# fmidev/RoadSurf

Measured on AMD Instinct MI355X. Metric: point_timesteps_per_s, higher is better.
Workload: dtype f64

## Files before the change

### roadsurf_amd/csrc/rs_api.hip

```cpp
#include <hip/hip_runtime.h>
#include <atomic>
#include <cmath>
#include <cstdarg>
#include <cstdio>
#include <cstdlib>
#include <cstring>
#include <mutex>
#include <utility>
#include <vector>

#include "../../include/roadsurf.h"
#include "rs_kernels.h"
#include "rs_devutil.hpp"
#include <cstdint>
#include <algorithm>
#include "rs_consts_dev.h"
#include "rs_state.h"

static thread_local char g_err[512] = "";

static int set_err(const char *fmt, ...) {
  va_list ap;
  va_start(ap, fmt);
  vsnprintf(g_err, sizeof(g_err), fmt, ap);
// ... 28 lines not shown
  double *relax_tab = nullptr;
  double *cpl_tab = nullptr;
  void *consts32_dev = nullptr;
  rs::Writeback wb{nullptr, nullptr, nullptr, 0};
  int32_t *cpl_flags = nullptr, *cpl_list = nullptr, *cpl_count = nullptr;
  void *cpl_tmp = nullptr;
  size_t cpl_tmp_bytes = 0;
  int32_t cpl_rounds_last = 0;
  bool output_by_point = false;
  bool cpl_windows_closed = false;
  bool history_score = true;
  bool f32 = false;
  double *diag = nullptr;
  bool diag_on = false;
  bool resorted = false;
  int32_t *wave_tab = nullptr;
  int32_t wave_n = 0;
  bool wave_tab_valid = false;
  std::vector<void *> owned;
  rsu::Arena *arena = nullptr;
  uint64_t arena_epoch = 0;
  bool arena_set = false;
  std::vector<hipEvent_t> ev;
  size_t ev_used = 0;
  bool timing = false;
};

template <class T>
static hipError_t plan_malloc(RsPlan *pl, T **p, size_t bytes) {
  rsu::Arena *a = rsu::tls_arena();
// ... 203 lines not shown

static inline int32_t underfilled(const RsPlan *pl) {
  return g_live_points[pl->device & 63].load() <= 131072 ? 1 : 0;
}

void rs_hip_plan_destroy(RsPlan *pl) {
  if (!pl) return;
  g_live_points[pl->device & 63] -= pl->npoints;
  (void)hipSetDevice(pl->device);
  (void)hipStreamSynchronize(pl->stream);
  for (hipEvent_t e : pl->ev) (void)hipEventDestroy(e);
  for (void *q : pl->owned) (void)hipFree(q);
  delete pl;
}

const int32_t *rs_hip_plan_order(RsPlan *pl) {
  if (!pl) {
    set_err("rs_hip_plan_order: null plan");
    return nullptr;
  }
  if (!pl->order) {
    if (hipSetDevice(pl->device) != hipSuccess ||
        plan_malloc(pl, &pl->order, pl->np_pad * sizeof(int32_t)) != hipSuccess ||
        rs_cluster_identity(pl->order, pl->np_pad, pl->stream) != hipSuccess) {
      set_err("rs_hip_plan_order: allocation failed");
      return nullptr;
    }
  }
  return pl->order;
}

static int recluster_buffers(RsPlan *pl) {
  const size_t state_bytes = (size_t)RS_NSTATE * pl->np_pad * sizeof(double);
  if (!pl->state_alt) {
    HIP_OK(plan_malloc(pl, &pl->state_alt, state_bytes));
    HIP_OK(plan_malloc(pl, &pl->order_alt, pl->np_pad * sizeof(int32_t)));
    HIP_OK(plan_malloc(pl, &pl->sort_keys, (size_t)4 * pl->np_pad * sizeof(uint32_t)));
    pl->sort_tmp_bytes = std::max(rs_cluster_scratch_bytes(pl->npoints),
                                  rs_cluster_count_scratch_bytes(pl->npoints, 12));
    HIP_OK(plan_malloc(pl, &pl->sort_tmp, pl->sort_tmp_bytes ? pl->sort_tmp_bytes : 8));
  }
  return 0;
}

static int recluster_apply(RsPlan *pl) {
  pl->resorted = true;
  HIP_OK(rs_cluster_apply(pl->state, pl->state_alt, pl->f32, pl->order, pl->order_alt,
                          pl->sort_keys + 3 * pl->np_pad, pl->np_pad, pl->npoints, pl->c.NLayers,
                          pl->c.use_coupling == 0 ? 0 : pl->cpl_windows_closed ? 1 : 2, pl->stream));
  std::swap(pl->state, pl->state_alt);
  std::swap(pl->order, pl->order_alt);
  return 0;
}

int rs_hip_recluster_forecast(RsPlan *pl, const RsPreview *pv) {
  if (!pl || !pv) return set_err("rs_hip_recluster_forecast: bad arguments");
  if (pv->n < 1 || pv->n > RS_PREVIEW_MAX || (!pv->tair_now && !pv->tair_b[0]))
    return set_err("rs_hip_recluster_forecast: 1 <= n <= %d previews and tair_now (or a preview 0 between two rows) are required",
                   RS_PREVIEW_MAX);
  for (int q = 0; q < pv->n; ++q) {
    if (!pv->tair[q] || !pv->vz[q]) return set_err("rs_hip_recluster_forecast: preview row %d is null", q);
    if ((pv->tair_b[q] != nullptr) != (pv->vz_b[q] != nullptr) || (pv->tair_b[q] && !(pv->w[q] >= 0.0 && pv->w[q] <= 1.0)))
      return set_err("rs_hip_recluster_forecast: preview %d: tair_b and vz_b come together, with 0 <= w <= 1", q);
  }
  if (pl->diag_on)
    return set_err("rs_hip_recluster_forecast: a plan with diagnostics keeps its order (rs_hip_set_diagnostics)");
// ... 30 lines not shown
        HIP_OK(plan_malloc(pl, &pl->wave_tab, ((size_t)2 * maxw + 64) * sizeof(int32_t)));
        pl->wave_n = maxw;
        HIP_OK(hipMemsetAsync(pl->wave_tab + 2 * (size_t)maxw, 0, 64 * sizeof(int32_t), pl->stream));
      }
      class_total = reinterpret_cast<uint32_t *>(pl->wave_tab + 2 * (size_t)maxw);
    }
    HIP_OK(rs_cluster_count_sort(pl->np_pad, pl->npoints, bits, pl->sort_keys, pl->sort_tmp,
                                 pl->sort_tmp_bytes, pl->stream, class_total, cb, low));
    if (table) {
      HIP_OK(rs_cluster_wave_table(cb, class_total, pl->wave_tab, pl->wave_tab + maxw, maxw, pl->stream));
      pl->wave_tab_valid = true;
    }
  } else
    HIP_OK(rs_cluster_sort_keys(pl->np_pad, pl->npoints, pl->sort_keys, pl->sort_tmp, pl->sort_tmp_bytes,
                                pl->stream));
  return recluster_apply(pl);
}

int rs_hip_recluster(RsPlan *pl) {
  if (!pl) return set_err("rs_hip_recluster: null plan");
  if (!pl->history_score)
    return set_err("rs_hip_recluster: the plan's history score is switched off (rs_hip_set_history_score)");
  if (pl->diag_on) return set_err("rs_hip_recluster: a plan with diagnostics keeps its order (rs_hip_set_diagnostics)");
  if (!rs_hip_plan_order(pl)) return -1;
  pl->wave_tab_valid = false;
  HIP_OK(hipSetDevice(pl->device));
  if (recluster_buffers(pl)) return -1;
  HIP_OK(rs_cluster_sort(pl->state, pl->f32, pl->np_pad, pl->npoints, pl->sort_keys, pl->sort_tmp,
                         pl->sort_tmp_bytes, pl->stream));
  return recluster_apply(pl);
}

int rs_hip_plan_order_copy(RsPlan *pl, int32_t *dst) {
  if (!pl || !dst) return set_err("rs_hip_plan_order_copy: bad arguments");
  if (!rs_hip_plan_order(pl)) return -1;
  HIP_OK(hipSetDevice(pl->device));
  HIP_OK(hipMemcpyAsync(dst, pl->order, (size_t)pl->np_pad * sizeof(int32_t), hipMemcpyDeviceToDevice,
                        pl->stream));
  return 0;
}

int rs_hip_outputs_by_point(RsPlan *pl, const RsOutputs *src, int32_t nrows, const int32_t *order,
                            double *const *dst, int64_t dst_rows, int64_t dst_row0, void *stream) {
  if (!pl || !src || !dst || nrows < 1 || dst_rows < 1 || dst_row0 < 0 || dst_row0 + nrows > dst_rows)
    return set_err("rs_hip_outputs_by_point: bad arguments (rows [dst_row0, dst_row0 + nrows) must lie inside a point's dst_rows)");
  if (pl->f32) return set_err("rs_hip_outputs_by_point: fp64 output windows only");
  const double *in[6] = {src->tsurf, src->snow, src->water, src->ice, src->deposit, src->ice2};
  double *out[6];
  for (int f = 0; f < 6; ++f) {
    if (!in[f] || !dst[f]) return set_err("rs_hip_outputs_by_point: all six streams are required on both sides");
    out[f] = dst[f];
  }
  if (src->t_stride < pl->npoints) return set_err("rs_hip_outputs_by_point: t_stride below the plan's points");
  if (!order && stream) return set_err("rs_hip_outputs_by_point: on a stream of the caller's the order row must be a kept one");
  if (!order && !rs_hip_plan_order(pl)) return -1;
  HIP_OK(hipSetDevice(pl->device));
  HIP_OK(rs_cluster_outputs_by_point(in, out, order ? order : pl->order, pl->npoints, src->t_stride, nrows, dst_rows,
                                     dst_row0, stream ? (hipStream_t)stream : pl->stream));
  return 0;
}

int rs_hip_plan_reset_order(RsPlan *pl) {
  if (!pl) return set_err("rs_hip_plan_reset_order: null plan");
  pl->wave_tab_valid = false;
  if (!pl->order) return rs_hip_plan_order(pl) ? 0 : -1;
  HIP_OK(hipSetDevice(pl->device));
  HIP_OK(rs_cluster_identity(pl->order, pl->np_pad, pl->stream));
  pl->resorted = false;
  return 0;
}

int64_t rs_hip_plan_npoints(const RsPlan *pl) { return pl ? pl->npoints : 0; }
int64_t rs_hip_plan_npoints_padded(const RsPlan *pl) { return pl ? pl->np_pad : 0; }
size_t rs_hip_plan_state_bytes(const RsPlan *pl) {
  return pl ? (size_t)RS_NSTATE * pl->np_pad * sizeof(double) : 0;
}

int rs_hip_set_precision(RsPlan *pl, int32_t bits) {
  if (!pl || (bits != 32 && bits != 64)) return set_err("rs_hip_set_precision: bits must be 32 or 64");
  HIP_OK(hipSetDevice(pl->device));
  if (bits == 32) {
    if (!pl->consts32_dev) HIP_OK(plan_malloc(pl, &pl->consts32_dev, rs32_constants_bytes()));
    HIP_OK(rs32_upload_constants(pl->consts32_dev, &pl->c, pl->stream));
  }
  pl->f32 = (bits == 32);
  return 0;
}

int rs_hip_set_writeback(RsPlan *pl, double *sw, double *sw_dir, double *lw, int64_t t_stride) {
  if (!pl) return set_err("rs_hip_set_writeback: null plan");
  if ((sw || sw_dir || lw) && (!sw || !sw_dir || !lw || t_stride < pl->npoints))
    return set_err("rs_hip_set_writeback: all three streams and t_stride >= npoints, or all NULL");
  pl->wb = rs::Writeback{sw, sw_dir, lw, t_stride};
  return 0;
}

int rs_hip_set_diagnostics(RsPlan *pl, int32_t on) {
  if (!pl) return set_err("rs_hip_set_diagnostics: null plan");
  if (on && pl->f32) return set_err("rs_hip_set_diagnostics: the fp64 flavour only");
  if (on && pl->resorted)
    return set_err("rs_hip_set_diagnostics: the block is kept by slot - not for a plan that has been re-sorted");
  HIP_OK(hipSetDevice(pl->device));
  if (on) {
    const size_t bytes = (size_t)RS_DIAG_ROWS * pl->np_pad * sizeof(double);
    if (!pl->diag) HIP_OK(plan_malloc(pl, &pl->diag, bytes));
    HIP_OK(hipMemsetAsync(pl->diag, 0, bytes, pl->stream));
  }
  pl->diag_on = on != 0;
  return 0;
}

int rs_hip_diagnostics(RsPlan *pl, double *out) {
  if (!pl || !out) return set_err("rs_hip_diagnostics: bad arguments");
  if (!pl->diag_on || !pl->diag) return set_err("rs_hip_diagnostics: rs_hip_set_diagnostics(plan, 1) first");
  HIP_OK(hipSetDevice(pl->device));
  std::vector<double> rows((size_t)(RS_DIAG_ROWS + 1) * pl->np_pad);
  HIP_OK(hipMemcpyAsync(rows.data(), pl->diag, (size_t)RS_DIAG_ROWS * pl->np_pad * sizeof(double), hipMemcpyDeviceToHost,
                        pl->stream));
  HIP_OK(hipMemcpyAsync(rows.data() + (size_t)RS_DIAG_ROWS * pl->np_pad, pl->state + (size_t)RS_ST_CPL_FLAGS * pl->np_pad,
                        (size_t)pl->np_pad * sizeof(double), hipMemcpyDeviceToHost, pl->stream));
  HIP_OK(hipStreamSynchronize(pl->stream));
  for (int64_t p = 0; p < pl->npoints; ++p) {
    for (int r = 0; r < RS_DIAG_ROWS; ++r) out[(size_t)p * RS_DIAG_COLS + r] = rows[(size_t)r * pl->np_pad + p];
    const int32_t fl = (int32_t)rows[(size_t)RS_DIAG_ROWS * pl->np_pad + p];
    out[(size_t)p * RS_DIAG_COLS + RS_DIAG_ROWS] = (double)(fl & (RS_CPL_MSG_SMALL | RS_CPL_MSG_BIG));
  }
  return 0;
}

int rs_hip_set_output_by_point(RsPlan *pl, int32_t on) {
  if (!pl) return set_err("rs_hip_set_output_by_point: null plan");
  pl->output_by_point = on != 0;
  return 0;
}

int rs_hip_coupling_windows_closed(RsPlan *pl, int32_t closed) {
  if (!pl) return set_err("rs_hip_coupling_windows_closed: null plan");
  pl->cpl_windows_closed = closed != 0;
  return 0;
}

int rs_hip_set_history_score(RsPlan *pl, int32_t on) {
  if (!pl) return set_err("rs_hip_set_history_score: null plan");
  pl->history_score = on != 0;
  return 0;
}

int rs_hip_set_variant(RsPlan *pl, int32_t variant) {
  if (!pl || variant < 0 || variant > 4) return set_err("rs_hip_set_variant: the flavour is 0 (automatic) ... 4");
  if (variant == RS_VARIANT_REG && pl->c.NLayers != 15)
    return set_err("register-profile kernel is built for NLayers == 15 only (got %d)",
                   pl->c.NLayers);
// ... 1 lines not shown
  return 0;
}

static int check_forcing(const RsPlan *pl, const RsForcing *f, const char *who) {
  if (!f || !f->tair || !f->vz || !f->rhz || !f->prec || !f->sw || !f->lw || !f->precphase ||
      !f->hour)
    return set_err("%s: forcing streams tair,vz,rhz,prec,sw,lw,precphase,hour are required", who);
  if (f->t_stride < pl->npoints)
    return set_err("%s: forcing t_stride %lld < npoints %lld", who, (long long)f->t_stride,
                   (long long)pl->npoints);
  return 0;
}

int rs_hip_init_state(RsPlan *pl, const RsForcing *f, const RsPointParams *pp) {
  if (!pl) return set_err("rs_hip_init_state: null plan");
  if (check_forcing(pl, f, "rs_hip_init_state")) return -1;
  if (!pp || !pp->tbottom) return set_err("rs_hip_init_state: tbottom is required");
  HIP_OK(hipSetDevice(pl->device));
  rs::InitArgs a;
  a.consts = pl->f32 ? pl->consts32_dev : pl->consts_dev;
  a.f = *f;
  a.pp = *pp;
  a.state = pl->state;
  a.npoints = pl->npoints;
  a.np_pad = pl->np_pad;
  pl->cpl_windows_closed = false;
  if (pl->f32) {
    HIP_OK(rs32_launch_init(a, pl->stream));
  } else {
    HIP_OK(rs_launch_init(a, pl->stream));
// ... 39 lines not shown
      HIP_OK(rs_cpl_select_again(pl->state, pl->np_pad, pl->npoints, pl->cpl_flags, pl->cpl_list,
                                 pl->cpl_count, pl->cpl_tmp, pl->cpl_tmp_bytes, pl->stream));
      HIP_OK(hipMemcpyAsync(&n_again, pl->cpl_count, sizeof(n_again), hipMemcpyDeviceToHost, pl->stream));
      HIP_OK(hipStreamSynchronize(pl->stream));
      if (n_again != 0)
        return set_err("coupling replays: %d points still ask for a replay after 64 rounds - the window "
                       "passed does not cover their coupling windows", n_again);
    }
  }
  return 0;
}

int rs_hip_step(RsPlan *pl, const RsForcing *f, const RsOutputs *o, const RsPointParams *pp,
                int32_t t0, int32_t nsteps) {
  if (!pl) return set_err("rs_hip_step: null plan");
  if (check_forcing(pl, f, "rs_hip_step")) return -1;
  if (!pp || !pp->tbottom) return set_err("rs_hip_step: tbottom is required");
  if (!o || !o->tsurf || !o->snow || !o->water || !o->ice || !o->deposit || !o->ice2)
    return set_err("rs_hip_step: all six output streams are required");
  if (o->t_stride < pl->npoints) return set_err("rs_hip_step: output t_stride < npoints");
  if (o->decimate < 1) return set_err("rs_hip_step: decimate must be >= 1");
  if (t0 < 1 || nsteps < 1 || (int64_t)t0 + nsteps - 1 > pl->c.SimLen)
    return set_err("rs_hip_step: window [%d,%d) outside [1,SimLen=%d]", t0, t0 + nsteps,
                   pl->c.SimLen);
  {
    const int64_t first = ((int64_t)t0 - 1 + o->decimate - 1) / o->decimate;
    if (first < o->row0) return set_err("rs_hip_step: output row0 %lld beyond first row %lld",
                                        (long long)o->row0, (long long)first);
  }
  HIP_OK(hipSetDevice(pl->device));
// ... 44 lines not shown
  a.duo_full_ok = (full && !skyview && !coupled && !f->depth && !(pl->c.tsurfOutputDepth >= 0.0)) ? 1 : 0;
  {
    const int64_t orows = ((int64_t)t0 + nsteps - 2) / o->decimate - o->row0 + 1;
    const bool a32 = (uint64_t)f->t_stride * (uint64_t)nsteps < rs_a32_limit() &&
                     (uint64_t)o->t_stride * (uint64_t)(orows > 0 ? orows : 1) < rs_a32_limit() &&
                     (!pl->wb.sw_dir || (uint64_t)pl->wb.t_stride * (uint64_t)nsteps < rs_a32_limit());
    if (skyview && !coupled && !f->depth && !(pl->c.tsurfOutputDepth >= 0.0) && a32) a.duo_full_ok |= 4;
  }
  a.surface_prio = underfilled(pl);
  a.knots = nullptr;
  a.knot_gather = nullptr;
  a.knot_k0 = a.knot_n = a.spk = a.start_hour = 0;
  a.r_spk = 0.0;
  std::memset(&a.raw, 0, sizeof(a.raw));
  a.diag = pl->diag_on ? pl->diag : nullptr;
  hipEvent_t e0 = nullptr, e1 = nullptr;
  if (pl->timing) {
    if (pl->ev_used + 2 > pl->ev.size()) {
      hipEvent_t x, y;
      HIP_OK(hipEventCreate(&x));
      if (hipEventCreate(&y) != hipSuccess) {
        (void)hipEventDestroy(x);
        return set_err("rs_hip_step: hipEventCreate failed");
      }
      pl->ev.push_back(x);
      pl->ev.push_back(y);
    }
    e0 = pl->ev[pl->ev_used];
    e1 = pl->ev[pl->ev_used + 1];
    HIP_OK(hipEventRecord(e0, pl->stream));
// ... 43 lines not shown
    const int32_t klast = tlast / spk + ((tlast % spk) ? 1 : 0);
    if (kfirst < k0 || klast >= k0 + nknots)
      return set_err("rs_hip_step_knots: need knots %d..%d, buffer has %d..%d", kfirst, klast, k0, k0 + nknots - 1);
    const int64_t first = ((int64_t)t0 - 1 + o->decimate - 1) / o->decimate;
    if (first < o->row0) return set_err("rs_hip_step_knots: output row0 beyond first row");
  }
  const int64_t out_rows = ((int64_t)t0 + nsteps - 2) / o->decimate - o->row0 + 1;
  if (pl->c.NLayers != 15 || pl->c.tsurfOutputDepth >= 0.0 || pp->sky_view ||
      (pl->c.use_coupling && pp->coupling_index) ||
      (!pl->f32 && (uint64_t)o->t_stride * (uint64_t)(out_rows > 0 ? out_rows : 1) >= rs_a32_limit()))
    return set_err("rs_hip_step_knots: NLayers = 15, no output depth, sky view or coupling and (fp64) an output "
                   "window below 4 GiB per stream only - use rs_hip_expand_forcing_ordered + rs_hip_step");
  const bool full = (pp->initlen != nullptr) || pl->c.force_tsurf || (pl->c.use_relaxation && pp->tair_relax != nullptr);
  if (pl->c.use_relaxation && pp->tair_relax && (!pp->vz_relax || !pp->rh_relax || !pp->initlen))
    return set_err("rs_hip_step_knots: relaxation needs tair_relax, vz_relax, rh_relax and initlen");
  const int32_t *order = rs_hip_plan_order(pl);
  if (!order) return -1;
  HIP_OK(hipSetDevice(pl->device));
  rs::StepArgs a;
  std::memset(&a, 0, sizeof(a));
  a.consts = pl->f32 ? pl->consts32_dev : pl->consts_dev;
  a.f.t_stride = pl->np_pad;
  a.o = *o;
  a.pp = *pp;
  a.state = pl->state;
  a.npoints = pl->npoints;
  a.np_pad = pl->np_pad;
  a.t0 = t0;
  a.nsteps = nsteps;
  a.wave_start = pl->wave_tab_valid ? pl->wave_tab : nullptr;
  a.wave_cnt = pl->wave_tab_valid ? pl->wave_tab + pl->wave_n : nullptr;
  a.wave_n = pl->wave_n;
  a.duo_full_ok = full ? 3 : 0;
  a.surface_prio = underfilled(pl);
  a.knots = knots;
  a.knot_gather = order;
  a.knot_k0 = k0;
  a.knot_n = nknots;
  a.spk = spk;
  a.start_hour = spec->start_hour;
  a.r_spk = 1.0 / (double)spk;
  a.diag = nullptr;
  hipEvent_t e0 = nullptr, e1 = nullptr;
  if (pl->timing) {
    if (pl->ev_used + 2 > pl->ev.size()) {
      hipEvent_t x, y;
      HIP_OK(hipEventCreate(&x));
      if (hipEventCreate(&y) != hipSuccess) {
        (void)hipEventDestroy(x);
        return set_err("rs_hip_step_knots: hipEventCreate failed");
      }
      pl->ev.push_back(x);
      pl->ev.push_back(y);
    }
    e0 = pl->ev[pl->ev_used];
    e1 = pl->ev[pl->ev_used + 1];
    HIP_OK(hipEventRecord(e0, pl->stream));
  }
  const hipError_t le = pl->f32 ? rs32_launch_step_knots(a, pl->history_score, full, pl->stream)
                                : rs_launch_step_duo_knots(a, pl->history_score, pl->stream);
  if (le != hipSuccess) return set_err("rs_hip_step_knots: kernel launch failed: %s", hipGetErrorString(le));
  if (pl->timing) {
    HIP_OK(hipEventRecord(e1, pl->stream));
    pl->ev_used += 2;
  }
  return 0;
}

}

int rs_step_raw(RsPlan *pl, const rs::RawForcing *raw, const double *sun, const RsOutputs *o,
                const RsPointParams *pp, int32_t t0, int32_t nsteps, bool out_by_point) {
  if (!pl || !raw || raw->nsrc < 1 || raw->nsrc > RS_MAX_SOURCES || !raw->segs || !raw->hour)
    return set_err("rs_step_raw: bad arguments");
  if (!pp || !pp->tbottom || !pp->initlen) return set_err("rs_step_raw: tbottom and initlen are required");
  if (!o || !o->tsurf || !o->snow || !o->water || !o->ice || !o->deposit || !o->ice2)
    return set_err("rs_step_raw: all six output streams are required");
  if (o->t_stride < pl->npoints || o->decimate < 1) return set_err("rs_step_raw: bad output window");
  if (t0 < 1 || nsteps < 1 || (int64_t)t0 + nsteps - 1 > pl->c.SimLen)
    return set_err("rs_step_raw: window [%d,%d) outside [1,SimLen=%d]", t0, t0 + nsteps, pl->c.SimLen);
  const int64_t first = ((int64_t)t0 - 1 + o->decimate - 1) / o->decimate;
  if (first < o->row0) return set_err("rs_step_raw: output row0 beyond first row");
  const int64_t out_rows = ((int64_t)t0 + nsteps - 2) / o->decimate - o->row0 + 1;
  if (!rs_step_raw_ok(pl) || (uint64_t)o->t_stride * (uint64_t)(out_rows > 0 ? out_rows : 1) >= rs_a32_limit())
    return set_err("rs_step_raw: NLayers = 15, fp64, no output depth and an output window below 4 GiB per stream only");
  const bool coupled = pl->c.use_coupling != 0;
  if (coupled && (!pp->coupling_index || !pp->coupling_tsurf))
    return set_err("rs_step_raw: use_coupling is set: pass coupling_index and coupling_tsurf");
  if (pl->c.use_relaxation && pp->tair_relax && (!pp->vz_relax || !pp->rh_relax))
// ... 20 lines not shown
  a.wave_n = pl->wave_n;
  a.duo_full_ok = 3;
  a.surface_prio = underfilled(pl);
  a.raw = *raw;
  a.diag = nullptr;
  a.out_index = (out_by_point && pl->order) ? pl->order : nullptr;
  const hipError_t le = rs_launch_step_duo_raw(a, pl->history_score, sky, coupled, pl->stream);
  if (le != hipSuccess) return set_err("rs_step_raw: kernel launch failed: %s", hipGetErrorString(le));
  return 0;
}

int rs_cpl_replay_raw(RsPlan *pl, const rs::RawForcing *raw, const RsOutputs *o, const RsPointParams *pp,
                      int32_t t0, int32_t nsteps, bool out_by_point, int32_t *rounds) {
  if (!pl || !raw || raw->nsrc < 1 || raw->nsrc > RS_MAX_SOURCES || !raw->segs || !raw->hour)
    return set_err("rs_cpl_replay_raw: bad arguments");
  if (!pp || !pp->tbottom || !pp->initlen || !pp->coupling_index || !pp->coupling_tsurf)
    return set_err("rs_cpl_replay_raw: tbottom, initlen, coupling_index and coupling_tsurf are required");
  if (!pl->c.use_coupling || !rs_step_raw_ok(pl) || pp->sky_view)
    return set_err("rs_cpl_replay_raw: a coupled plan with NLayers = 15, fp64, no output depth, no sky view only");
  if (!o || !o->tsurf || !o->snow || !o->water || !o->ice || !o->deposit || !o->ice2 || o->decimate < 1)
    return set_err("rs_cpl_replay_raw: all six output streams are required");
  if (t0 < 1 || nsteps < 1 || (int64_t)t0 + nsteps - 1 >= pl->c.SimLen)
    return set_err("rs_cpl_replay_raw: the block [%d,%d] must lie inside [1, SimLen - 1]", t0, t0 + nsteps - 1);
  const int64_t out_rows = ((int64_t)t0 + nsteps - 2) / o->decimate - o->row0 + 1;
  if ((uint64_t)o->t_stride * (uint64_t)(out_rows > 0 ? out_rows : 1) >= rs_a32_limit())
    return set_err("rs_cpl_replay_raw: output window of 4 GiB per stream or more");
  if (raw->seg0 < 0 || raw->seg0 >= raw->nseg) return set_err("rs_cpl_replay_raw: seg0 outside the segment table");
  HIP_OK(hipSetDevice(pl->device));
  rs::StepArgs a;
  std::memset(&a, 0, sizeof(a));
// ... 29 lines not shown
  }
  if (cpl_replay_rounds(pl, a, true, true)) return -1;
  if (rounds) *rounds = pl->cpl_rounds_last;
  return 0;
}

bool rs_step_raw_ok(const RsPlan *pl) {
  return pl && !pl->f32 && pl->c.NLayers == 15 && !(pl->c.tsurfOutputDepth >= 0.0);
}

extern "C" {

static int cpl_args(RsPlan *pl, const RsForcing *f, const RsOutputs *o, const RsPointParams *pp,
                    int32_t t0, int32_t nsteps, const char *who, rs::StepArgs &a) {
  if (!pl) return set_err("%s: null plan", who);
  if (check_forcing(pl, f, who)) return -1;
  if (!pp || !pp->tbottom || !pp->coupling_index || !pp->coupling_tsurf)
    return set_err("%s: tbottom, coupling_index and coupling_tsurf are required", who);
  if (!pl->c.use_coupling) return set_err("%s: the plan's settings have use_coupling = 0", who);
  if (pl->f32) return set_err("%s: time-chunked coupling needs the fp64 flavour (an fp32 plan runs a coupled series whole: rs_hip_step)", who);
  if (pp->sky_view) {
    if (!pp->sin_lat || !pp->cos_lat || !pp->lon_rad || !f->sw_dir || !f->lw_net || !f->sun)
      return set_err("%s: sky view needs sin_lat, cos_lat, lon_rad, sw_dir, lw_net and sun", who);
    if (f->hour_pstride) return set_err("%s: sky view needs a time axis shared by all points", who);
    if (pl->wb.sw_dir)
      return set_err("%s: the write-back of the sky-view edits follows whole-series windows: use "
                     "rs_hip_step", who);
  }
  if (pl->c.use_relaxation && pp->tair_relax && (!pp->vz_relax || !pp->rh_relax || !pp->initlen))
    return set_err("%s: relaxation needs tair_relax, vz_relax, rh_relax and initlen", who);
// ... 15 lines not shown
  a.cpl_list = nullptr;
  a.cpl_nlist = 0;
  a.cpl_stop = 0;
  a.cpl_inner = a.cpl_prio = 0;
  a.out_index = (pl->output_by_point && pl->order) ? pl->order : nullptr;
  a.wave_start = a.wave_cnt = nullptr;
  a.wave_n = 0;
  a.duo_full_ok = 0;
  a.surface_prio = 0;
  a.diag = nullptr;
  a.knots = nullptr;
  a.knot_gather = nullptr;
  a.knot_k0 = a.knot_n = a.spk = a.start_hour = 0;
  a.r_spk = 0.0;
  std::memset(&a.raw, 0, sizeof(a.raw));
  return 0;
}

int rs_hip_step_cpl(RsPlan *pl, const RsForcing *f, const RsOutputs *o, const RsPointParams *pp,
                    int32_t t0, int32_t nsteps) {
  rs::StepArgs a;
  if (cpl_args(pl, f, o, pp, t0, nsteps, "rs_hip_step_cpl", a)) return -1;
  HIP_OK(hipSetDevice(pl->device));
  HIP_OK(rs_launch_step_cpl(a, pl->c.NLayers, pl->stream));
  return 0;
}

int rs_hip_cpl_replay(RsPlan *pl, const RsForcing *f, const RsOutputs *o, const RsPointParams *pp,
                      int32_t t0, int32_t nsteps, int32_t *rounds) {
  rs::StepArgs a;
// ... 61 lines not shown
  if (hipEventSynchronize(pl->ev[pl->ev_used - 1]) != hipSuccess) return -1;
  for (int32_t i = 0; i < n && i < cap; ++i) {
    float a = 0.f, b = 0.f;
    if (hipEventElapsedTime(&a, (hipEvent_t)ref_event, pl->ev[2 * (size_t)i]) != hipSuccess ||
        hipEventElapsedTime(&b, (hipEvent_t)ref_event, pl->ev[2 * (size_t)i + 1]) != hipSuccess)
      return set_err("rs_hip_timing_intervals: hipEventElapsedTime failed");
    start_ms[i] = a;
    stop_ms[i] = b;
  }
  return n;
}

int rs_hip_state_download(RsPlan *pl, double *host, size_t bytes) {
  if (!pl || !host || bytes != rs_hip_plan_state_bytes(pl))
    return set_err("rs_hip_state_download: bad arguments");
  HIP_OK(hipSetDevice(pl->device));
  HIP_OK(hipMemcpyAsync(host, pl->state, bytes, hipMemcpyDeviceToHost, pl->stream));
  HIP_OK(hipStreamSynchronize(pl->stream));
  return 0;
}

int rs_hip_state_upload(RsPlan *pl, const double *host, size_t bytes) {
  if (!pl || !host || bytes != rs_hip_plan_state_bytes(pl))
    return set_err("rs_hip_state_upload: bad arguments");
  HIP_OK(hipSetDevice(pl->device));
  HIP_OK(hipMemcpyAsync(pl->state, host, bytes, hipMemcpyHostToDevice, pl->stream));
  HIP_OK(hipStreamSynchronize(pl->stream));
  return 0;
}

int rs_hip_clock_probe(int32_t device, void *out, uint32_t spin_us, void *stream) {
  if (!out) return set_err("rs_hip_clock_probe: null output");
  HIP_OK(hipSetDevice(device));
  HIP_OK(rs_launch_clock_probe(static_cast<uint64_t *>(out), spin_us, (hipStream_t)stream));
  return 0;
}

int64_t rs_hip_failed_count(RsPlan *pl) {
  if (!pl) return -1;
  if (hipSetDevice(pl->device) != hipSuccess) return -1;
  unsigned long long h = 0;
  if (pl->f32) {
    std::vector<float> row((size_t)pl->np_pad);
    if (hipMemcpyAsync(row.data(), (const char *)pl->state + (size_t)RS_ST_FAILED * pl->np_pad * sizeof(float),
                       row.size() * sizeof(float), hipMemcpyDeviceToHost, pl->stream) != hipSuccess)
      return -1;
    if (hipStreamSynchronize(pl->stream) != hipSuccess) return -1;
    for (int64_t q = 0; q < pl->npoints; ++q) h += row[(size_t)q] != 0.f ? 1 : 0;
    return (int64_t)h;
  }
  if (hipMemsetAsync(pl->counter, 0, sizeof(h), pl->stream) != hipSuccess) return -1;
  if (rs_launch_count_failed(pl->state, pl->np_pad, pl->npoints, pl->counter, pl->stream) !=
      hipSuccess)
    return -1;
  if (hipMemcpyAsync(&h, pl->counter, sizeof(h), hipMemcpyDeviceToHost, pl->stream) != hipSuccess)
    return -1;
  if (hipStreamSynchronize(pl->stream) != hipSuccess) return -1;
  return (int64_t)h;
}

int rs_hip_first_failed_index(RsPlan *pl, int32_t *out) {
  if (!pl || !out) return set_err("rs_hip_first_failed_index: bad arguments");
  HIP_OK(hipSetDevice(pl->device));
  const size_t esz = pl->f32 ? sizeof(float) : sizeof(double);
  std::vector<char> row((size_t)pl->np_pad * esz);
  HIP_OK(hipMemcpyAsync(row.data(), (const char *)pl->state + (size_t)RS_ST_FAILED * pl->np_pad * esz,
                        row.size(), hipMemcpyDeviceToHost, pl->stream));
  std::vector<int32_t> order;
  if (pl->order) {
    order.resize((size_t)pl->np_pad);
    HIP_OK(hipMemcpyAsync(order.data(), pl->order, order.size() * sizeof(int32_t), hipMemcpyDeviceToHost,
                          pl->stream));
  }
  HIP_OK(hipStreamSynchronize(pl->stream));
  for (int64_t s = 0; s < pl->npoints; ++s) {
    const double v = pl->f32 ? (double)reinterpret_cast<const float *>(row.data())[s]
                             : reinterpret_cast<const double *>(row.data())[s];
// ... 44 lines not shown
  return 1;
#endif
}

int rs_hip_test_math(RsPlan *pl, int32_t fn, int64_t n, const double *x, double *y) {
  if (!pl || !x || !y || n < 1 || fn < 0 || fn > 3) return set_err("rs_hip_test_math: bad arguments");
  HIP_OK(hipSetDevice(pl->device));
  HIP_OK(rs_launch_math_test(fn, n, x, y, pl->stream));
  return 0;
}

int rs_hip_synth_knots(RsPlan *pl, const RsSynthSpec *spec, double *knots, int32_t k0,
                       int32_t nknots) {
  if (!pl || !spec || !knots || nknots < 1 || k0 < 0)
    return set_err("rs_hip_synth_knots: bad arguments");
  if (nknots > 65535) return set_err("rs_hip_synth_knots: at most 65535 knots per call");
  HIP_OK(hipSetDevice(pl->device));
  rs::KnotArgs a;
  a.spec = *spec;
  a.knots = knots;
  a.npoints = pl->npoints;
  a.np_pad = pl->np_pad;
  a.k0 = k0;
  HIP_OK(rs_launch_knots(a, nknots, pl->stream));
  return 0;
}

static int expand_forcing(RsPlan *pl, const RsSynthSpec *spec, const double *knots, int32_t k0,
                          int32_t nknots, const RsForcing *f, int32_t t0, int32_t nsteps, void *stream,
                          const int32_t *gather) {
// ... 58 lines not shown
```

### roadsurf_amd/csrc/rs_kernels.h

```cpp
#pragma once
#include <hip/hip_runtime.h>
#include "../../include/roadsurf.h"
#include "rs_synth.h"
#include "rs_raw.hpp"

#define RS_BLOCK 256

enum { RS_VARIANT_AUTO = 0, RS_VARIANT_REG = 1, RS_VARIANT_LDS = 2, RS_VARIANT_DUO = 3, RS_VARIANT_HYBRID = 4 };
#ifndef RS_DUO_MAX_POINTS
#define RS_DUO_MAX_POINTS 65536
#endif

namespace rs {

struct Writeback {
  double *sw, *sw_dir, *lw;
  int64_t t_stride;
};

struct StepArgs {
  const void *consts;
  RsForcing f;
  RsOutputs o;
  RsPointParams pp;
// ... 3 lines not shown
  Writeback wb;
  const int32_t *cpl_list;
  int32_t cpl_nlist, cpl_stop;
  int32_t cpl_inner, cpl_prio;
  const int32_t *out_index;
  const int32_t *wave_start, *wave_cnt;
  int32_t wave_n;
  int32_t duo_full_ok;
  int32_t surface_prio;
  const double *knots;
  const int32_t *knot_gather;
  int32_t knot_k0, knot_n, spk, start_hour;
  double r_spk;
  RawForcing raw;
  double *diag;
};

struct InitArgs {
  const void *consts;
  RsForcing f;
  RsPointParams pp;
  double *state;
  int64_t npoints, np_pad;
};

struct ForecastArgs {
  const void *consts;
  const void *state;
  int32_t f32;
  int64_t npoints, np_pad;
// ... 95 lines not shown
```

### roadsurf_amd/csrc/rs_kernels.hip

```cpp
#include <hip/hip_runtime.h>
#include <cstdlib>
#include "rs_physics.hpp"
#include "rs_state.h"
#include "rs_synth.h"
#include "rs_kernels.h"

#ifndef RS_CPL_WAVES
#define RS_CPL_WAVES 2
#endif
#ifndef RS_REGIME_WINDOW
#define RS_REGIME_WINDOW 30
#endif

namespace rs {

constexpr int kBlock = RS_BLOCK;

typedef RsConstantsDev __attribute__((address_space(4))) ConstsAS;
template <class Args>
__device__ __forceinline__ const ConstsAS &consts_of(Args a) {
  return *(const ConstsAS *)a->consts;
}

template <int NL>
// ... 1063 lines not shown
    q.trffric = q.night ? fricN : fricD;
  }
  q.PsychC = R4(0.1) * (R4(0.00063) * (q.tair + R4(273.15)) + R4(0.47496));
  q.den0 = AirVCap * (q.tair + R4(273.15));
  q.vkvz = c.VK_Const * q.vz;
  q.avk = AirVCap * c.VK_Const;
  q.bad = (flags & 1u) != 0u;
  q.stop = SKYG && (flags & 4u) != 0u;
  q.bad_rw = (flags & 8u) != 0u;
  return q;
}

__device__ __forceinline__ void duo_meet() { asm volatile("s_waitcnt lgkmcnt(0)\n\ts_barrier" ::: "memory"); }

template <int NL, bool SCORE, bool FULL = false, bool SKY = false, bool SKYG = false, bool OUTIDX = false,
          bool CPL = false, bool REPLAY = false>
__device__ __forceinline__ void duo_surface(const MathTab &mt, DuoMailT<FULL ? PR_FULL : PR_LEAN> &mail, const StepArgs &a,
                                            const uint32_t *skyfl = nullptr) {
  static_assert(FULL || !SKY, "sky view belongs to the FULL feature set");
  static_assert(!(SKY && SKYG), "the sky view is this wave's or the ground wave's");
  static_assert(FULL || !CPL, "coupling belongs to the FULL feature set");
  static_assert(CPL || !REPLAY, "replays belong to coupling");
  KernArgs ka = kernargs();
  const uint32_t ml = threadIdx.x & 63u;
  const int64_t listed = REPLAY ? (int64_t)blockIdx.x * 64 + ml : 0;
  const int64_t row0 = REPLAY ? 0 : a.wave_start ? (int64_t)a.wave_start[blockIdx.x] : (int64_t)blockIdx.x * 64;
  const uint32_t lane = REPLAY ? (listed < a.cpl_nlist ? (uint32_t)a.cpl_list[listed] : 0u) : ml;
  const int64_t p = row0 + lane;
  const bool live = REPLAY ? listed < a.cpl_nlist
                           : a.wave_start ? (int32_t)lane < a.wave_cnt[blockIdx.x] : p < a.npoints;
  RegProfile<2> T;
  Scalars s;
  {
    RegProfile<NL> all;
    if (live) {
      load_state<false>(a.state, a.np_pad, p, all, s);
    } else {
      for (int j = 1; j <= NL; ++j) all.set(j, 0.0);
      s = Scalars();
      s.failed = true;
    }
    T.set(1, all.get(1));
    T.set(2, all.get(2));
  }
  double skyv = R4(1.0), sinlat = 0, coslat = 0, lonrad = 0, coslon = 1.0, sinlon = 0;
  bool sky_on = false;
  uint32_t hcol = 0;
  if (SKY && live) {
    skyv = ka->pp.sky_view[p];
    sky_on = (skyv < R4(1.0) && skyv > R4(-0.01));
    if (sky_on) {
// ... 500 lines not shown
template <int NL, int SRC = SRC_WINDOW, bool FULL = false, bool SKYG = false, bool CPL = false, bool REPLAY = false>
__device__ __forceinline__ void duo_ground(const MathTab &mt, DuoMailT<FULL ? PR_FULL : PR_LEAN> &mail, const StepArgs &a) {
  constexpr bool KNOTS = SRC == SRC_KNOTS, RAW = SRC == SRC_RAW;
  static_assert(FULL || !CPL, "coupling belongs to the FULL feature set");
  static_assert(!RAW || FULL, "the driver's series carry the FULL feature set");
  static_assert(!SKYG || RAW, "a sky wave exists only where the forcing is made from the raw series");
  static_assert(!REPLAY || (CPL && RAW && !SKYG), "replay rounds in this flavour: raw series, no sky view");
  KernArgs ka = kernargs();
  const uint32_t ml = threadIdx.x & 63u;
  const int64_t listed = REPLAY ? (int64_t)blockIdx.x * 64 + ml : 0;
  const int64_t row0 = REPLAY ? 0 : a.wave_start ? (int64_t)a.wave_start[blockIdx.x] : (int64_t)blockIdx.x * 64;
  const uint32_t lane = REPLAY ? (listed < a.cpl_nlist ? (uint32_t)a.cpl_list[listed] : 0u) : ml;
  const int64_t p = row0 + lane;
  const bool live = REPLAY ? listed < a.cpl_nlist
                           : a.wave_start ? (int32_t)lane < a.wave_cnt[blockIdx.x] : p < a.npoints;
  double Tg[NL - 2];
#pragma unroll
  for (int j = 3; j <= NL; ++j) Tg[j - 3] = live ? a.state[(int64_t)(RS_ST_TMP0 + j - 1) * a.np_pad + p] : 0.0;
  const double tbot = live ? ka->pp.tbottom[p] : 0.0;
  mail.v[0][1][ml] = Tg[0];
  const int32_t nsteps = ka->nsteps, t0 = ka->t0;
  int32_t initlen = 0;
  bool relax = false;
  double relax_dt = 0, relax_dv = 0, relax_dr = 0;
  auto relax_targets = [&](double &tairR, double &vzR, double &rhR) {
    tairR = (double)(float)ka->pp.tair_relax[p];
    vzR = (double)(float)ka->pp.vz_relax[p];
    rhR = (double)(float)ka->pp.rh_relax[p];
  };
  if (FULL && live) {
    initlen = ka->pp.initlen ? ka->pp.initlen[p] : 0;
    if (consts_of(ka).use_relaxation && ka->pp.tair_relax) {
      double tairR, vzR, rhR;
// ... 61 lines not shown
      const int32_t tb = cpl_ce;
      g.tair = ka->raw.status && ka->raw.status[rcol_] != 0 ? raw_miss() : raw_slow_value(ka, RAW_TAIR, rcol_, tb);
      g.vz = raw_slow_value(ka, RAW_VZ, rcol_, tb);
      g.rhz = raw_slow_value(ka, RAW_RHZ, rcol_, tb);
      g.prec = raw_slow_value(ka, RAW_PREC, rcol_, tb);
      g.sw = raw_slow_value(ka, RAW_SW, rcol_, tb);
      g.lw = raw_slow_value(ka, RAW_LW, rcol_, tb);
      g.tdew = raw_slow_value(ka, RAW_TDEW, rcol_, tb);
      q.bad_rw = check_values_forcing(c, g) | (g.tdew < -90) | (g.tdew > R4(100.0));
    }
    return q;
  };
  Forcing nxt = Forcing();
  KnotLerp<FULL> klerp;
  int32_t kcur = -1;
  const int64_t kcol = (KNOTS && live) ? (ka->knot_gather ? (int64_t)ka->knot_gather[p] : p) : 0;
  constexpr int FSET = SKYG ? FSET_GROUND : FSET_ALL;
  RawLerp<raw_nfields(FSET)> rlerp;
  const int64_t rcol = rcol_;
  const bool rejected = RAW && live && ka->raw.status && ka->raw.status[rcol] != 0;
  auto obs_wanted = [&](const ConstsAS &c, int32_t in) -> bool {
    return c.force_tsurf || __builtin_amdgcn_ballot_w64(live && in <= initlen) != 0ull;
  };
  if (RAW) {
    rlerp.seg = ka->raw.seg0;
    raw_resolve<FSET>(ka, rcol, live, rlerp);
  }
  {
    const ConstsAS &c0 = consts_of(ka);
    if (KNOTS) nxt = knot_forcing<FULL>(ka, kcol, live, klerp, kcur, t0);
    else if (RAW) nxt = raw_forcing<FSET>(ka, rcol, live, rejected, rlerp, t0, obs_wanted(c0, t0));
// ... 121 lines not shown
          bool REPLAY = false>
#ifndef RS_DUO_LEAN_WAVES
#define RS_DUO_LEAN_WAVES 4
#endif
__global__ void __launch_bounds__((SKY && SRC == SRC_RAW) ? 192 : 128, REPLAY ? 3 : FULL ? 4 : RS_DUO_LEAN_WAVES) step_kernel_duo(const StepArgs a) {
  static_assert(!CPL || SRC == SRC_RAW, "coupling in the two-wavefront flavour: the driver path's lock-step chunks");
  constexpr bool SKYG = SKY && SRC == SRC_RAW;
  __shared__ double math_lds[RS_MATH_LDS_DOUBLES];
  __shared__ DuoMailT<FULL ? PR_FULL : PR_LEAN> mail;
  __shared__ uint32_t skyfl[SKYG ? 2 * 64 : 1];
  const MathTab mt = fill_math_tables(math_lds);
  __syncthreads();
  if (a.wave_start && a.wave_cnt[blockIdx.x] == 0) return;
  if (threadIdx.x < 64) {
    if (a.surface_prio) __builtin_amdgcn_s_setprio(1);
    duo_surface<NL, SCORE, FULL, SKY && !SKYG, SKYG, SRC == SRC_RAW, CPL, REPLAY>(mt, mail, a, skyfl);
  } else if (!SKYG || threadIdx.x < 128) {
    duo_ground<NL, SRC, FULL, SKYG, CPL, REPLAY>(mt, mail, a);
  } else {
    if constexpr (SKYG) duo_sky(mail, skyfl, a);
  }
}

template <bool DIAG = false>
__global__ void __launch_bounds__(kBlock, 3) step_kernel_sky(const StepArgs a) {
  extern __shared__ double lds[];
  __shared__ double math_lds[RS_MATH_LDS_DOUBLES];
  const MathTab mt = fill_math_tables(math_lds);
  __syncthreads();
  const int64_t p = (int64_t)blockIdx.x * kBlock + threadIdx.x;
  if (p >= a.npoints) return;
// ... 722 lines not shown
```

Baseline: 24.89 billion.

## Fuse recluster state permutation into the next knots step kernel

After a re-sort, the state permutation (gather into the alternate buffer) is deferred and folded into the next knots step kernel. That kernel loads each point's state from its source slot and writes the order array, instead of running a separate apply pass over the whole state. Every other API entry point first settles any pending permutation. This removes one full read and write of the state between recluster and step, at the cost of gathered, uncoalesced loads inside the step kernel and more bookkeeping.

Measured after the change: 25.05 billion (median of 6 runs). About the same (+0.6%).

```diff
diff --git a/roadsurf_amd/csrc/rs_api.hip b/roadsurf_amd/csrc/rs_api.hip
--- a/roadsurf_amd/csrc/rs_api.hip
+++ b/roadsurf_amd/csrc/rs_api.hip
@@ -66,6 +66,7 @@
   double *diag = nullptr;
   bool diag_on = false;
   bool resorted = false;
+  bool perm_pending = false;
   int32_t *wave_tab = nullptr;
   int32_t wave_n = 0;
   bool wave_tab_valid = false;
@@ -299,11 +300,7 @@
   delete pl;
 }
 
-const int32_t *rs_hip_plan_order(RsPlan *pl) {
-  if (!pl) {
-    set_err("rs_hip_plan_order: null plan");
-    return nullptr;
-  }
+static const int32_t *order_buf(RsPlan *pl) {
   if (!pl->order) {
     if (hipSetDevice(pl->device) != hipSuccess ||
         plan_malloc(pl, &pl->order, pl->np_pad * sizeof(int32_t)) != hipSuccess ||
@@ -315,11 +312,36 @@
   return pl->order;
 }
 
+static int recluster_apply(RsPlan *pl);
+
+static int settle_order(RsPlan *pl) {
+  if (!pl->perm_pending) return 0;
+  pl->perm_pending = false;
+  HIP_OK(hipSetDevice(pl->device));
+  return recluster_apply(pl);
+}
+
+static bool resort_deferred(const RsPlan *pl) {
+  const char *e = getenv("ROADSURF_HIP_UNFUSED_RESORT");
+  if (e && *e && std::strcmp(e, "0") != 0) return false;
+  return !pl->f32 && pl->c.NLayers == 15 && pl->c.use_coupling == 0 && !pl->diag_on;
+}
+
+const int32_t *rs_hip_plan_order(RsPlan *pl) {
+  if (!pl) {
+    set_err("rs_hip_plan_order: null plan");
+    return nullptr;
+  }
+  if (settle_order(pl)) return nullptr;
+  return order_buf(pl);
+}
+
 static int recluster_buffers(RsPlan *pl) {
   const size_t state_bytes = (size_t)RS_NSTATE * pl->np_pad * sizeof(double);
   if (!pl->state_alt) {
     HIP_OK(plan_malloc(pl, &pl->state_alt, state_bytes));
     HIP_OK(plan_malloc(pl, &pl->order_alt, pl->np_pad * sizeof(int32_t)));
+    HIP_OK(rs_cluster_identity(pl->order_alt, pl->np_pad, pl->stream));
     HIP_OK(plan_malloc(pl, &pl->sort_keys, (size_t)4 * pl->np_pad * sizeof(uint32_t)));
     pl->sort_tmp_bytes = std::max(rs_cluster_scratch_bytes(pl->npoints),
                                   rs_cluster_count_scratch_bytes(pl->npoints, 12));
@@ -335,6 +357,13 @@
                           pl->c.use_coupling == 0 ? 0 : pl->cpl_windows_closed ? 1 : 2, pl->stream));
   std::swap(pl->state, pl->state_alt);
   std::swap(pl->order, pl->order_alt);
+  return 0;
+}
+
+static int recluster_finish(RsPlan *pl) {
+  if (!resort_deferred(pl)) return recluster_apply(pl);
+  pl->resorted = true;
+  pl->perm_pending = true;
   return 0;
 }
 
@@ -395,7 +424,7 @@
   } else
     HIP_OK(rs_cluster_sort_keys(pl->np_pad, pl->npoints, pl->sort_keys, pl->sort_tmp, pl->sort_tmp_bytes,
                                 pl->stream));
-  return recluster_apply(pl);
+  return recluster_finish(pl);
 }
 
 int rs_hip_recluster(RsPlan *pl) {
@@ -409,11 +438,12 @@
   if (recluster_buffers(pl)) return -1;
   HIP_OK(rs_cluster_sort(pl->state, pl->f32, pl->np_pad, pl->npoints, pl->sort_keys, pl->sort_tmp,
                          pl->sort_tmp_bytes, pl->stream));
-  return recluster_apply(pl);
+  return recluster_finish(pl);
 }
 
 int rs_hip_plan_order_copy(RsPlan *pl, int32_t *dst) {
   if (!pl || !dst) return set_err("rs_hip_plan_order_copy: bad arguments");
+  if (settle_order(pl)) return -1;
   if (!rs_hip_plan_order(pl)) return -1;
   HIP_OK(hipSetDevice(pl->device));
   HIP_OK(hipMemcpyAsync(dst, pl->order, (size_t)pl->np_pad * sizeof(int32_t), hipMemcpyDeviceToDevice,
@@ -425,6 +455,7 @@
                             double *const *dst, int64_t dst_rows, int64_t dst_row0, void *stream) {
   if (!pl || !src || !dst || nrows < 1 || dst_rows < 1 || dst_row0 < 0 || dst_row0 + nrows > dst_rows)
     return set_err("rs_hip_outputs_by_point: bad arguments (rows [dst_row0, dst_row0 + nrows) must lie inside a point's dst_rows)");
+  if (settle_order(pl)) return -1;
   if (pl->f32) return set_err("rs_hip_outputs_by_point: fp64 output windows only");
   const double *in[6] = {src->tsurf, src->snow, src->water, src->ice, src->deposit, src->ice2};
   double *out[6];
@@ -443,6 +474,7 @@
 
 int rs_hip_plan_reset_order(RsPlan *pl) {
   if (!pl) return set_err("rs_hip_plan_reset_order: null plan");
+  if (settle_order(pl)) return -1;
   pl->wave_tab_valid = false;
   if (!pl->order) return rs_hip_plan_order(pl) ? 0 : -1;
   HIP_OK(hipSetDevice(pl->device));
@@ -459,6 +491,7 @@
 
 int rs_hip_set_precision(RsPlan *pl, int32_t bits) {
   if (!pl || (bits != 32 && bits != 64)) return set_err("rs_hip_set_precision: bits must be 32 or 64");
+  if (settle_order(pl)) return -1;
   HIP_OK(hipSetDevice(pl->device));
   if (bits == 32) {
     if (!pl->consts32_dev) HIP_OK(plan_malloc(pl, &pl->consts32_dev, rs32_constants_bytes()));
@@ -478,6 +511,7 @@
 
 int rs_hip_set_diagnostics(RsPlan *pl, int32_t on) {
   if (!pl) return set_err("rs_hip_set_diagnostics: null plan");
+  if (settle_order(pl)) return -1;
   if (on && pl->f32) return set_err("rs_hip_set_diagnostics: the fp64 flavour only");
   if (on && pl->resorted)
     return set_err("rs_hip_set_diagnostics: the block is kept by slot - not for a plan that has been re-sorted");
@@ -493,6 +527,7 @@
 
 int rs_hip_diagnostics(RsPlan *pl, double *out) {
   if (!pl || !out) return set_err("rs_hip_diagnostics: bad arguments");
+  if (settle_order(pl)) return -1;
   if (!pl->diag_on || !pl->diag) return set_err("rs_hip_diagnostics: rs_hip_set_diagnostics(plan, 1) first");
   HIP_OK(hipSetDevice(pl->device));
   std::vector<double> rows((size_t)(RS_DIAG_ROWS + 1) * pl->np_pad);
@@ -517,6 +552,7 @@
 
 int rs_hip_coupling_windows_closed(RsPlan *pl, int32_t closed) {
   if (!pl) return set_err("rs_hip_coupling_windows_closed: null plan");
+  if (settle_order(pl)) return -1;
   pl->cpl_windows_closed = closed != 0;
   return 0;
 }
@@ -548,6 +584,7 @@
 
 int rs_hip_init_state(RsPlan *pl, const RsForcing *f, const RsPointParams *pp) {
   if (!pl) return set_err("rs_hip_init_state: null plan");
+  if (settle_order(pl)) return -1;
   if (check_forcing(pl, f, "rs_hip_init_state")) return -1;
   if (!pp || !pp->tbottom) return set_err("rs_hip_init_state: tbottom is required");
   HIP_OK(hipSetDevice(pl->device));
@@ -617,6 +654,7 @@
 int rs_hip_step(RsPlan *pl, const RsForcing *f, const RsOutputs *o, const RsPointParams *pp,
                 int32_t t0, int32_t nsteps) {
   if (!pl) return set_err("rs_hip_step: null plan");
+  if (settle_order(pl)) return -1;
   if (check_forcing(pl, f, "rs_hip_step")) return -1;
   if (!pp || !pp->tbottom) return set_err("rs_hip_step: tbottom is required");
   if (!o || !o->tsurf || !o->snow || !o->water || !o->ice || !o->deposit || !o->ice2)
@@ -691,6 +729,9 @@
   a.r_spk = 0.0;
   std::memset(&a.raw, 0, sizeof(a.raw));
   a.diag = pl->diag_on ? pl->diag : nullptr;
+  a.state_src = nullptr;
+  a.perm = nullptr;
+  a.order_dst = nullptr;
   hipEvent_t e0 = nullptr, e1 = nullptr;
   if (pl->timing) {
     if (pl->ev_used + 2 > pl->ev.size()) {
@@ -764,7 +805,9 @@
   const bool full = (pp->initlen != nullptr) || pl->c.force_tsurf || (pl->c.use_relaxation && pp->tair_relax != nullptr);
   if (pl->c.use_relaxation && pp->tair_relax && (!pp->vz_relax || !pp->rh_relax || !pp->initlen))
     return set_err("rs_hip_step_knots: relaxation needs tair_relax, vz_relax, rh_relax and initlen");
-  const int32_t *order = rs_hip_plan_order(pl);
+  const bool move = pl->perm_pending && !pl->f32 && !full;
+  if (!move && settle_order(pl)) return -1;
+  const int32_t *order = order_buf(pl);
   if (!order) return -1;
   HIP_OK(hipSetDevice(pl->device));
   rs::StepArgs a;
@@ -791,6 +834,12 @@
   a.start_hour = spec->start_hour;
   a.r_spk = 1.0 / (double)spk;
   a.diag = nullptr;
+  if (move) {
+    a.state_src = pl->state;
+    a.state = pl->state_alt;
+    a.perm = pl->sort_keys + 3 * pl->np_pad;
+    a.order_dst = pl->order_alt;
+  }
   hipEvent_t e0 = nullptr, e1 = nullptr;
   if (pl->timing) {
     if (pl->ev_used + 2 > pl->ev.size()) {
@@ -810,6 +859,11 @@
   const hipError_t le = pl->f32 ? rs32_launch_step_knots(a, pl->history_score, full, pl->stream)
                                 : rs_launch_step_duo_knots(a, pl->history_score, pl->stream);
   if (le != hipSuccess) return set_err("rs_hip_step_knots: kernel launch failed: %s", hipGetErrorString(le));
+  if (move) {
+    std::swap(pl->state, pl->state_alt);
+    std::swap(pl->order, pl->order_alt);
+    pl->perm_pending = false;
+  }
   if (pl->timing) {
     HIP_OK(hipEventRecord(e1, pl->stream));
     pl->ev_used += 2;
@@ -823,6 +877,7 @@
                 const RsPointParams *pp, int32_t t0, int32_t nsteps, bool out_by_point) {
   if (!pl || !raw || raw->nsrc < 1 || raw->nsrc > RS_MAX_SOURCES || !raw->segs || !raw->hour)
     return set_err("rs_step_raw: bad arguments");
+  if (settle_order(pl)) return -1;
   if (!pp || !pp->tbottom || !pp->initlen) return set_err("rs_step_raw: tbottom and initlen are required");
   if (!o || !o->tsurf || !o->snow || !o->water || !o->ice || !o->deposit || !o->ice2)
     return set_err("rs_step_raw: all six output streams are required");
@@ -873,6 +928,7 @@
                       int32_t t0, int32_t nsteps, bool out_by_point, int32_t *rounds) {
   if (!pl || !raw || raw->nsrc < 1 || raw->nsrc > RS_MAX_SOURCES || !raw->segs || !raw->hour)
     return set_err("rs_cpl_replay_raw: bad arguments");
+  if (settle_order(pl)) return -1;
   if (!pp || !pp->tbottom || !pp->initlen || !pp->coupling_index || !pp->coupling_tsurf)
     return set_err("rs_cpl_replay_raw: tbottom, initlen, coupling_index and coupling_tsurf are required");
   if (!pl->c.use_coupling || !rs_step_raw_ok(pl) || pp->sky_view)
@@ -932,6 +988,7 @@
 static int cpl_args(RsPlan *pl, const RsForcing *f, const RsOutputs *o, const RsPointParams *pp,
                     int32_t t0, int32_t nsteps, const char *who, rs::StepArgs &a) {
   if (!pl) return set_err("%s: null plan", who);
+  if (settle_order(pl)) return -1;
   if (check_forcing(pl, f, who)) return -1;
   if (!pp || !pp->tbottom || !pp->coupling_index || !pp->coupling_tsurf)
     return set_err("%s: tbottom, coupling_index and coupling_tsurf are required", who);
@@ -977,6 +1034,9 @@
   a.knot_k0 = a.knot_n = a.spk = a.start_hour = 0;
   a.r_spk = 0.0;
   std::memset(&a.raw, 0, sizeof(a.raw));
+  a.state_src = nullptr;
+  a.perm = nullptr;
+  a.order_dst = nullptr;
   return 0;
 }
 
@@ -1068,6 +1128,7 @@
 int rs_hip_state_download(RsPlan *pl, double *host, size_t bytes) {
   if (!pl || !host || bytes != rs_hip_plan_state_bytes(pl))
     return set_err("rs_hip_state_download: bad arguments");
+  if (settle_order(pl)) return -1;
   HIP_OK(hipSetDevice(pl->device));
   HIP_OK(hipMemcpyAsync(host, pl->state, bytes, hipMemcpyDeviceToHost, pl->stream));
   HIP_OK(hipStreamSynchronize(pl->stream));
@@ -1077,6 +1138,7 @@
 int rs_hip_state_upload(RsPlan *pl, const double *host, size_t bytes) {
   if (!pl || !host || bytes != rs_hip_plan_state_bytes(pl))
     return set_err("rs_hip_state_upload: bad arguments");
+  if (settle_order(pl)) return -1;
   HIP_OK(hipSetDevice(pl->device));
   HIP_OK(hipMemcpyAsync(pl->state, host, bytes, hipMemcpyHostToDevice, pl->stream));
   HIP_OK(hipStreamSynchronize(pl->stream));
@@ -1092,6 +1154,7 @@
 
 int64_t rs_hip_failed_count(RsPlan *pl) {
   if (!pl) return -1;
+  if (settle_order(pl)) return -1;
   if (hipSetDevice(pl->device) != hipSuccess) return -1;
   unsigned long long h = 0;
   if (pl->f32) {
@@ -1115,6 +1178,7 @@
 
 int rs_hip_first_failed_index(RsPlan *pl, int32_t *out) {
   if (!pl || !out) return set_err("rs_hip_first_failed_index: bad arguments");
+  if (settle_order(pl)) return -1;
   HIP_OK(hipSetDevice(pl->device));
   const size_t esz = pl->f32 ? sizeof(float) : sizeof(double);
   std::vector<char> row((size_t)pl->np_pad * esz);
@@ -1189,6 +1253,7 @@
                        int32_t nknots) {
   if (!pl || !spec || !knots || nknots < 1 || k0 < 0)
     return set_err("rs_hip_synth_knots: bad arguments");
+  if (settle_order(pl)) return -1;
   if (nknots > 65535) return set_err("rs_hip_synth_knots: at most 65535 knots per call");
   HIP_OK(hipSetDevice(pl->device));
   rs::KnotArgs a;
diff --git a/roadsurf_amd/csrc/rs_kernels.h b/roadsurf_amd/csrc/rs_kernels.h
--- a/roadsurf_amd/csrc/rs_kernels.h
+++ b/roadsurf_amd/csrc/rs_kernels.h
@@ -41,6 +41,9 @@
   double r_spk;
   RawForcing raw;
   double *diag;
+  const double *state_src;
+  const uint32_t *perm;
+  int32_t *order_dst;
 };
 
 struct InitArgs {
diff --git a/roadsurf_amd/csrc/rs_kernels.hip b/roadsurf_amd/csrc/rs_kernels.hip
--- a/roadsurf_amd/csrc/rs_kernels.hip
+++ b/roadsurf_amd/csrc/rs_kernels.hip
@@ -1101,7 +1101,7 @@
 __device__ __forceinline__ void duo_meet() { asm volatile("s_waitcnt lgkmcnt(0)\n\ts_barrier" ::: "memory"); }
 
 template <int NL, bool SCORE, bool FULL = false, bool SKY = false, bool SKYG = false, bool OUTIDX = false,
-          bool CPL = false, bool REPLAY = false>
+          bool CPL = false, bool REPLAY = false, bool MOVE = false>
 __device__ __forceinline__ void duo_surface(const MathTab &mt, DuoMailT<FULL ? PR_FULL : PR_LEAN> &mail, const StepArgs &a,
                                             const uint32_t *skyfl = nullptr) {
   static_assert(FULL || !SKY, "sky view belongs to the FULL feature set");
@@ -1121,7 +1121,13 @@
   {
     RegProfile<NL> all;
     if (live) {
-      load_state<false>(a.state, a.np_pad, p, all, s);
+      if (MOVE && a.perm) {
+        const int64_t from = (int64_t)a.perm[p];
+        load_state<false>(a.state_src, a.np_pad, from, all, s);
+        a.state[(int64_t)RS_ST_FAILED * a.np_pad + p] = a.state_src[(int64_t)RS_ST_FAILED * a.np_pad + from];
+      } else {
+        load_state<false>(a.state, a.np_pad, p, all, s);
+      }
     } else {
       for (int j = 1; j <= NL; ++j) all.set(j, 0.0);
       s = Scalars();
@@ -1652,9 +1658,18 @@
   const int64_t p = row0 + lane;
   const bool live = REPLAY ? listed < a.cpl_nlist
                            : a.wave_start ? (int32_t)lane < a.wave_cnt[blockIdx.x] : p < a.npoints;
+  constexpr bool MOVE = KNOTS && !FULL;
+  const bool moving = MOVE && a.perm != nullptr;
+  const int64_t from = (moving && live) ? (int64_t)a.perm[p] : p;
+  const double *const st_in = moving ? a.state_src : a.state;
   double Tg[NL - 2];
 #pragma unroll
-  for (int j = 3; j <= NL; ++j) Tg[j - 3] = live ? a.state[(int64_t)(RS_ST_TMP0 + j - 1) * a.np_pad + p] : 0.0;
+  for (int j = 3; j <= NL; ++j) Tg[j - 3] = live ? st_in[(int64_t)(RS_ST_TMP0 + j - 1) * a.np_pad + from] : 0.0;
+  if (moving && live) {
+#pragma unroll
+    for (int r = RS_ST_TAIR_END; r <= RS_ST_RH_END; ++r)
+      a.state[(int64_t)r * a.np_pad + p] = a.state_src[(int64_t)r * a.np_pad + from];
+  }
   const double tbot = live ? ka->pp.tbottom[p] : 0.0;
   mail.v[0][1][ml] = Tg[0];
   const int32_t nsteps = ka->nsteps, t0 = ka->t0;
@@ -1746,7 +1761,8 @@
   Forcing nxt = Forcing();
   KnotLerp<FULL> klerp;
   int32_t kcur = -1;
-  const int64_t kcol = (KNOTS && live) ? (ka->knot_gather ? (int64_t)ka->knot_gather[p] : p) : 0;
+  const int64_t kcol = (KNOTS && live) ? (ka->knot_gather ? (int64_t)ka->knot_gather[from] : from) : 0;
+  if (moving && live) a.order_dst[p] = (int32_t)kcol;
   constexpr int FSET = SKYG ? FSET_GROUND : FSET_ALL;
   RawLerp<raw_nfields(FSET)> rlerp;
   const int64_t rcol = rcol_;
@@ -1898,7 +1914,7 @@
   if (a.wave_start && a.wave_cnt[blockIdx.x] == 0) return;
   if (threadIdx.x < 64) {
     if (a.surface_prio) __builtin_amdgcn_s_setprio(1);
-    duo_surface<NL, SCORE, FULL, SKY && !SKYG, SKYG, SRC == SRC_RAW, CPL, REPLAY>(mt, mail, a, skyfl);
+    duo_surface<NL, SCORE, FULL, SKY && !SKYG, SKYG, SRC == SRC_RAW, CPL, REPLAY, SRC == SRC_KNOTS && !FULL>(mt, mail, a, skyfl);
   } else if (!SKYG || threadIdx.x < 128) {
     duo_ground<NL, SRC, FULL, SKYG, CPL, REPLAY>(mt, mail, a);
   } else {
```
